# TencentYoutuResearch/ImageMatching-OETR

Hardware: AMD Instinct MI355X
Metric: image-pairs/sec @640x640 (OETR hot path: feature correlation + overlap regression, features resident in HBM) (higher is better)
Workload: dtype f32 (3xf16-split operands, fp32 accumulate); 1 GPU; BASELINE configs[1]: batch=8 pairs/GPU, 640x640 -> 20x20 tokens/image, C=256, 8 enc + 2 dec layers, f32_split_f16; pairs_per_gpu=8, global_pairs=8, streams=3, world_size=1, gpu_max_hw_queues=4, encoder_tile_rows=64, tail_mode=direct form (throughput setting for overlapped streams), parallelism=pairs sharded over 1 rank(s); all-gather of boxes only

## Files before the change

### imagematching_oetr_amd/csrc/api.hip

```cpp
#include <math.h>
#include <stdlib.h>
#include <string.h>

#include <atomic>
#include <string>
#include <vector>

#include "../../include/oetr_hip.h"
#include "../../include/oetr_tail_share.h"
#include "common.h"

using namespace oetr;

constexpr int OETR_PREREDUCE_MIN_TOKENS = 768;
constexpr int OETR_DIRECT_TAIL_MIN_ROWS = 16000;

namespace {

thread_local std::string g_err;

oetr_status fail(oetr_status st, const std::string& msg) {
  g_err = msg;
  return st;
}
// ... 177 lines not shown
}

int encoder_tile_rows(const oetr_ctx* h, const Geom& g) {
  if (!gm_half(h->mode) || h->attn_full) return TM;
  const int want = h->enc_tile;
  if (want == TM || want == 64) return want;
  return g.ntiles > h->num_cus ? 64 : TM;
}
Geom encoder_geom(const Geom& g, int rows) {
  Geom e = g;
  for (int i = 0; i < 2; ++i) e.nt[i] = (g.L[i] + rows - 1) / rows;
  e.tile0[0] = 0; e.tile0[1] = g.N * e.nt[0];
  e.ntiles = g.N * (e.nt[0] + e.nt[1]);
  return e;
}

Workspace carve(const Geom& g, void* base, bool attn_full = false) {
  Workspace w;
  size_t off = 0;
  auto take = [&](size_t floats) {
    float* p = base ? reinterpret_cast<float*>(static_cast<char*>(base) + off) : nullptr;
    off += (floats * sizeof(float) + 255) & ~size_t(255);
    return p;
  };
  const size_t rows = g.rows, nt = g.ntiles;
  w.flags = reinterpret_cast<uint32_t*>(take(OETR_WORKSPACE_STATUS_BYTES / sizeof(float)));
  w.x = take(rows * C);
  w.qp = take((rows + (size_t)2 * g.N * 64) * C);
  w.pos = take((size_t)(g.L[0] + g.L[1]) * C);
  for (int i = 0; i < 2; ++i) { w.kvp[i] = take(nt * KV_FLOATS); w.ksp[i] = take(nt * C); }
  w.att0 = take(nt * C); w.z0 = take(nt * NH);
  w.dkv1 = take(nt * KV_FLOATS); w.dks1 = take(nt * C);
  w.conv_out = take(rows * C);
  w.gn_part = take(nt * 32 * 2);
  w.sm_part = take(nt * 4);
  w.hs = take((size_t)2 * g.N * C);
  w.logits = take(rows);
  w.cxy = take((size_t)2 * g.N * 2);
  w.tlbr = take((size_t)2 * g.N * 4);
  w.convp = take((size_t)9 * rows * C);
  w.kvr = take((size_t)2 * g.N * KV_FLOATS);
  w.ksr = take((size_t)2 * g.N * C);
  for (int i = 0; i < 2; ++i) {
    w.kbuf[i] = attn_full ? take(rows * C) : nullptr;
    w.vt[i] = attn_full ? take((size_t)g.N * C * TM * (g.nt[0] + g.nt[1])) : nullptr;
  }
  w.bytes = off;
  return w;
}

oetr_status check_ws(const Geom& g, void* ws, size_t ws_bytes, Workspace* out, bool attn_full = false) {
  if (!ws) return fail(OETR_ERR_WORKSPACE, "workspace is NULL");
  if (reinterpret_cast<uintptr_t>(ws) & 255)
    return fail(OETR_ERR_WORKSPACE, "workspace must be 256-byte aligned");
  *out = carve(g, ws, attn_full);
  if (out->bytes > ws_bytes)
    return fail(OETR_ERR_WORKSPACE, "workspace too small: need " + std::to_string(out->bytes) +
                                        " bytes, got " + std::to_string(ws_bytes));
  return OETR_OK;
}

HeatLaunch heat_launch(const oetr_ctx* h, const Geom& g, const Workspace& w, const float* mem1,
                       const float* mem2, const float* hs1, const float* hs2, float* cxy1,
                       float* cxy2, int img_h1, int img_h2) {
  HeatLaunch p;
  p.g = g;
  p.w = h->heads;
  p.mem[0] = mem1; p.mem[1] = mem2;
  p.hs[0] = hs1; p.hs[1] = hs2;
  p.conv_out = w.conv_out;
  p.gn_part = w.gn_part;
  p.sm_part = w.sm_part;
  p.logits = w.logits;
  p.cxy[0] = cxy1; p.cxy[1] = cxy2;
  p.img_h[0] = img_h1; p.img_h[1] = img_h2;
  p.tlbr[0] = p.tlbr[1] = nullptr;
  p.box[0] = p.box[1] = nullptr;
  p.img_w[0] = p.img_w[1] = 0;
  p.flags = w.flags;
  p.publish = nullptr;
  p.force_staged_conv = h->tail_mode == 3;
  p.convp_units = 9;
  p.mask[0] = p.mask[1] = nullptr;
  return p;
}

oetr_status check_masks(const oetr_ctx* h, const float* mask1, const float* mask2, bool encoder) {
  if (!mask1 && !mask2) return OETR_OK;
  if (!mask1 || !mask2) return fail(OETR_ERR_BAD_ARG, "masks: pass both mask1 and mask2, or neither");
  if (encoder && ((h->mode != GM_SPLIT && h->mode != GM_F32) || h->attn_full))
    return fail(OETR_ERR_UNSUPPORTED, "masks: built for OETR_DTYPE_F32_SPLIT_F16, OETR_DTYPE_F32_SPLIT_QK16 and OETR_DTYPE_F32 with linear attention "
                                      "(the reference's FullAttention turns a masked query row into NaN, "
                                      "linear_attention.py:74-81)");
  return OETR_OK;
}

struct Scoped {
  oetr_trace* t; hipStream_t s; int slot;
  Scoped(oetr_trace* tr, hipStream_t s_, int kid) : t(tr), s(s_), slot(-1) {
    if (!t) return;
    if (2 * (t->used + 1) > (int)t->ev.size()) { t->dropped++; t = nullptr; return; }
    slot = t->used++;
    t->kid[slot] = kid;
    (void)hipEventRecord(t->ev[2 * slot], s);
  }
  ~Scoped() { if (t) (void)hipEventRecord(t->ev[2 * slot + 1], s); }
};
#define TRACED(h, s, kid, expr)            \
  do {                                     \
    Scoped sc__((h)->trace, s, kid);       \
    HIP_TRY(expr);                         \
  } while (0)

DecLaunch dec_launch(const oetr_ctx* h, const Geom& g, const Workspace& w, bool beside_convp = false) {
  DecLaunch d;
  d.g = encoder_geom(g, encoder_tile_rows(h, g));
  for (int i = 0; i < 2; ++i) { d.layer[i] = h->dec[i]; d.qe[i] = h->qe[i]; }
  d.tgt1 = h->dec_tgt1; d.qkv1 = h->dec_qkv1;
  d.att0_part = w.att0; d.z0_part = w.z0; d.dkv1 = w.dkv1; d.dks1 = w.dks1;
  d.hs = w.hs;
  const int images = 2 * g.N;
  bool fits = images <= DEC_SPLIT_MAX_IMAGES && images * DEC_SPLIT_K * 4 <= h->num_cus;
  d.convp_units = 9;
  if (fits && beside_convp) {
    if (gm_half(h->mode)) {
      const int units = 9 * g.N * ((g.L[0] + RT - 1) / RT + (g.L[1] + RT - 1) / RT);
      const int avail = h->num_cus - images * DEC_SPLIT_K;
      const int upi = std::max(3, (units + avail - 1) / avail);
      fits = upi <= 9;
      if (fits) d.convp_units = upi;
    } else {
      fits = images * DEC_SPLIT_K + g.ntiles <= h->num_cus;
    }
  }
  if (h->dec_split == DEC_SPLIT_K && d.convp_units == 9 && beside_convp && gm_half(h->mode)) d.convp_units = 3;
  d.ksplit = (h->dec_split == DEC_SPLIT_K || (h->dec_split == 0 && fits)) && images <= DEC_SPLIT_MAX_IMAGES
                 ? DEC_SPLIT_K : 1;
  d.flags = w.flags;
  d.xch_epoch = w.flags + STATUS_EPOCH_WORD;
  d.xch = reinterpret_cast<unsigned long long*>(reinterpret_cast<char*>(w.flags) + STATUS_XCH_OFFSET);
  d.tbuf = nullptr;
  d.dbg = 0;
  if (d.ksplit == DEC_SPLIT_K && h->dec_fault) { d.dbg = DEC_DBG_FAULT; h->dec_fault = 0; }
#ifdef OETR_PHASE_TIMING
  d.tbuf = g_tbuf ? g_tbuf + 16 * 4096 : nullptr;
#endif
  return d;
}

oetr_status run_correlation(oetr_ctx* h, const Geom& g, const Workspace& w, const float* feat1,
                            const float* feat2, const float* pos1, const float* pos2,
                            int enc_layers, hipStream_t s, bool with_decoder = true,
                            bool resident = false, const float* mask1 = nullptr,
                            const float* mask2 = nullptr) {
  EncLaunch p;
  memset(&p, 0, sizeof(p));
  if (!resident) {
    p.feat_nchw[0] = feat1; p.feat_nchw[1] = feat2;
    p.pos_nchw[0] = pos1; p.pos_nchw[1] = pos2;
    p.pos_out = w.pos;
  }
  p.tile_rows = encoder_tile_rows(h, g);
  p.g = encoder_geom(g, p.tile_rows);
  p.tail_share = h->tail_share != 0;
  p.attn_full = h->attn_full;
  h->enc_grid.store(encoder_workgroups(p, h->mode), std::memory_order_relaxed);
// ... 1012 lines not shown
oetr_status oetr_debug_mfma_rate(int device, double seconds, double* tflops, void* stream) {
  if (!tflops || !(seconds > 0.0) || seconds > 30.0)
    return fail(OETR_ERR_BAD_ARG, "oetr_debug_mfma_rate: NULL output or seconds outside (0, 30]");
  int ndev = 0;
  if (hipGetDeviceCount(&ndev) != hipSuccess || ndev <= 0 || device < 0 || device >= ndev)
    return fail(OETR_ERR_NO_DEVICE, "no HIP device " + std::to_string(device));
  hipDeviceProp_t prop;
  HIP_TRY(hipGetDeviceProperties(&prop, device));
  int prev = 0;
  (void)hipGetDevice(&prev);
  hipError_t e = hipSetDevice(device);
  if (e == hipSuccess) e = measure_mfma_rate(prop.multiProcessorCount, seconds, tflops, static_cast<hipStream_t>(stream));
  (void)hipSetDevice(prev);
  if (e != hipSuccess) return hip_fail(e, "oetr_debug_mfma_rate");
  return OETR_OK;
}

oetr_status oetr_set_state_prereduce(oetr_handle h, int on) {
  if (!h) return fail(OETR_ERR_BAD_ARG, "oetr_set_state_prereduce: NULL handle");
  if (on < -1 || on > 1) return fail(OETR_ERR_BAD_ARG, "oetr_set_state_prereduce: -1 (auto), 0 (off) or 1 (a reduction launch between the encoder launches)");
  h->kv_prereduce = on;
  return OETR_OK;
}

oetr_status oetr_set_tail_share(oetr_handle h, int mode) {
  if (!h) return fail(OETR_ERR_BAD_ARG, "oetr_set_tail_share: NULL handle");
  if (mode != -1 && mode != 0) return fail(OETR_ERR_BAD_ARG, "oetr_set_tail_share: -1 (auto) or 0 (off)");
  h->tail_share = mode;
  return OETR_OK;
}

int oetr_debug_encoder_grid(oetr_handle h) { return h ? h->enc_grid.load(std::memory_order_relaxed) : -1; }

oetr_status oetr_set_attention(oetr_handle h, oetr_attention mode) {
  if (!h) return fail(OETR_ERR_BAD_ARG, "oetr_set_attention: NULL handle");
  if (mode != OETR_ATTENTION_LINEAR && mode != OETR_ATTENTION_FULL)
    return fail(OETR_ERR_BAD_ARG, "oetr_set_attention: unknown mode");
  if (mode == OETR_ATTENTION_FULL && h->policy != 0)
    return fail(OETR_ERR_UNSUPPORTED, "attention 'full' is not built for OETR_DTYPE_F32_SPLIT_QK16");
  if (mode == OETR_ATTENTION_FULL && !gm_f16_range(h->mode) && h->mode != GM_F32)
    return fail(OETR_ERR_UNSUPPORTED, "attention 'full' is built for OETR_DTYPE_F32_SPLIT_F16, OETR_DTYPE_F16 and OETR_DTYPE_F32");
  h->attn_full = mode == OETR_ATTENTION_FULL;
  return OETR_OK;
}

oetr_status oetr_set_trace(oetr_handle h, oetr_trace_handle t) {
  if (!h) return fail(OETR_ERR_BAD_ARG, "oetr_set_trace: NULL handle");
  h->trace = t;
  return OETR_OK;
}

oetr_status oetr_trace_summary(oetr_trace_handle t, int* n_kernels,
                               const char* names[OETR_TRACE_MAX_KERNELS],
                               int launches[OETR_TRACE_MAX_KERNELS],
                               float total_ms[OETR_TRACE_MAX_KERNELS]) {
  if (!t || !n_kernels || !names || !launches || !total_ms)
    return fail(OETR_ERR_BAD_ARG, "oetr_trace_summary: NULL argument");
  static_assert(K_COUNT <= OETR_TRACE_MAX_KERNELS, "raise OETR_TRACE_MAX_KERNELS");
  for (int i = 0; i < K_COUNT; ++i) { names[i] = kKernelNames[i]; launches[i] = 0; total_ms[i] = 0.f; }
  for (int i = 0; i < t->used; ++i) {
    HIP_TRY(hipEventSynchronize(t->ev[2 * i + 1]));
    float ms = 0.f;
    HIP_TRY(hipEventElapsedTime(&ms, t->ev[2 * i], t->ev[2 * i + 1]));
    launches[t->kid[i]]++;
    total_ms[t->kid[i]] += ms;
  }
  *n_kernels = K_COUNT;
  const int dropped = t->dropped;
  t->used = 0;
  t->dropped = 0;
  if (dropped) return fail(OETR_ERR_BAD_ARG, std::to_string(dropped) + " launches not traced: pool too small");
  return OETR_OK;
}

#ifdef OETR_PHASE_TIMING
int oetr_debug_read_tbuf(long long* host, int n_blocks) {
  if (!g_tbuf) return 1;
  return hipMemcpy(host, g_tbuf, sizeof(long long) * 16 * n_blocks, hipMemcpyDeviceToHost) != hipSuccess;
}
int oetr_debug_read_tbuf_decoder(long long* host, int n_blocks) {
  if (!g_tbuf) return 1;
  return hipMemcpy(host, g_tbuf + 16 * 4096, sizeof(long long) * 16 * n_blocks, hipMemcpyDeviceToHost) != hipSuccess;
}
#endif

}
```

### imagematching_oetr_amd/csrc/common.h

```cpp
#pragma once
#include <hip/hip_runtime.h>
#include <stdint.h>

#include <string>
#include <type_traits>

#include "../../include/oetr_hip.h"

namespace oetr {

constexpr int C = 256;
constexpr int NH = 8;
constexpr int HD = 32;
constexpr int FF = 512;
constexpr int TM = 32;
constexpr int LDA = C + 4;
constexpr int LDH = FF + 4;
constexpr int NTHREADS = 256;
constexpr int KV_FLOATS = NH * HD * HD;
constexpr float LN_EPS = 1e-5f;
constexpr float ATTN_EPS = 1e-6f;
constexpr int MAX_TOKENS = 10000;


// ... 831 lines not shown
  size_t vt_off[2];
  int tile_rows;
  int nwg;
  int tail_share;
  int b_cross;
  int kv_reduced;
  int policy;
  int dbg;
  long long* tbuf;
  uint32_t* flags;
  const float* feat_nchw[2];
  const float* pos_nchw[2];
  float* pos_out;
  const float* mask[2];
};

hipError_t launch_encoder(const EncLaunch& p, bool has_b, int tail, int mode, hipStream_t s);
int encoder_workgroups(const EncLaunch& p, int mode);
hipError_t launch_kv_reduce(const Geom& g, const float* kvp, const float* ksp, float* kvr, float* ksr,
                            hipStream_t s);

struct MhaDev {
  const float *wq_t, *wk_t, *wv_t, *wm_t;
  const float *bq, *bk, *bv;
};
struct DecLayerDev {
  MhaDev self_attn, cross;
  const float *w1_t, *w2_t;
  const float *n1w, *n1b, *n2w, *n2b, *n3w, *n3b;
};
struct DecLaunch {
  Geom g;
  DecLayerDev layer[2];
  const float* qe[2];
  const float* tgt1;
  const float* qkv1;
  const float* att0_part;
  const float* z0_part;
  const float* dkv1;
  const float* dks1;
  float* hs;
  int convp_units;
  int ksplit;
  unsigned long long* xch;
  unsigned* xch_epoch;
  uint32_t* flags;
  long long* tbuf;
  int dbg;
};
struct DecConstLaunch {
  DecLayerDev layer[2];
  const float* qe[2];
  float *tgt1, *q0, *qkv1;
};
hipError_t launch_decoder_consts(const DecConstLaunch& p, hipStream_t s);
hipError_t launch_decoder(const DecLaunch& p, hipStream_t s);

struct HeadsDev {
  const f32x4* conv_w;
  const f32x4* conv_w_l;
  const float *conv_b, *gn_w, *gn_b, *out_w, *out_b;
  const float *tlbr0_t;
  const float *tlbr2_w, *tlbr2_b;
};
struct HeatLaunch {
  Geom g;
  HeadsDev w;
  const float* mem[2];
  const float* hs[2];
  float* conv_out;
  float* gn_part;
  float* sm_part;
  float* logits;
  float* cxy[2];
  int img_h[2];
  float* tlbr[2];
  float* box[2];
  int img_w[2];
  uint32_t* flags;
  uint32_t* publish;
  int force_staged_conv;
  int convp_units;
  const float* mask[2];
};
hipError_t launch_heat_conv(const HeatLaunch& p, int mode, hipStream_t s);
hipError_t launch_heat_conv64(const HeatLaunch& p, int mode, hipStream_t s);
hipError_t launch_decoder_convp(const DecLaunch& d, const HeatLaunch& h, float* P, int mode,
                                hipStream_t s);
hipError_t launch_heat_combine(const HeatLaunch& h, const float* P, hipStream_t s);
hipError_t launch_heat_final(const HeatLaunch& p, hipStream_t s);
hipError_t launch_size_regression(const HeadsDev& w, const float* hs1, const float* hs2,
                                  int n, float* tlbr1, float* tlbr2, hipStream_t s);
hipError_t launch_boxes(const float* cxy, const float* tlbr, int n, int max_h, int max_w,
                        float* box, hipStream_t s);
constexpr int BBC = 1024;
constexpr int NECK_MT = 256;
constexpr int NECK_PIX = 16;
constexpr int NECK_XROW = 2 * C;
constexpr int NECK_RW_MIN_WO = 16;
struct NeckGeom {
  int n_img, hb, wb, ho, wo;
  int HW;
  int rows_in;
  int M;
};
struct NeckProjLaunch {
  NeckGeom g;
  const float* bb;
  const f32x4 *wh[2], *wl[2];
  const float *bias, *ln_w, *ln_b;
  _Float16 *xh, *xl;
  uint32_t* flags;
};
struct NeckConvDesc {
  const f32x4 *wh, *wl;
  const f32x4 *wh_rw, *wl_rw;
  float* part;
  int log2ks, pad, nsplit, nhalf, ncols;
  int item0;
};
struct NeckConvLaunch {
  NeckGeom g;
  const _Float16 *xh, *xl;
  NeckConvDesc conv[3];
  int items_per_mt;
  int mt_rows;
  int row_window;
  int nblocks;
};
struct NeckOutLaunch {
  NeckGeom g;
  const float* part[3];
  int nsplit[3];
  const float* bias[3];
  const f32x4 *wh, *wl;
  const float* bias2;
  float* feat;
  float* tokens;
  uint32_t* flags;
};
hipError_t launch_neck_proj(const NeckProjLaunch& p, hipStream_t s);
hipError_t launch_neck_conv(const NeckConvLaunch& p, hipStream_t s);
int neck_conv_rows(int M, int items_per_mt, int num_cus, int max_rows);
hipError_t launch_neck_out(const NeckOutLaunch& p, hipStream_t s);

hipError_t measure_mfma_rate(int num_cus, double seconds, double* tflops, hipStream_t s);

hipError_t launch_linear_attention(const float* q, const float* k, const float* v, const float* q_mask,
                                   const float* kv_mask, int n, int L, int S, float* out, float* state,
                                   hipStream_t s);
hipError_t launch_full_attention(const float* q, const float* k, const float* v, int n,
                                 int L, int S, float* out, hipStream_t s);
hipError_t launch_full_attention_split(const float* q, const float* k, const float* v, int n,
                                       int L, int S, float* out, uint32_t* flags, hipStream_t s);

}
```

### imagematching_oetr_amd/csrc/heads.hip

```cpp
#include "common.h"

namespace oetr {

constexpr int GN_GROUPS = 32;
constexpr float GN_EPS = 1e-5f;

template <int MODE, int NW>
__global__ __launch_bounds__(64 * NW) void k_heat_conv(HeatLaunch p) {
  constexpr int NT = 8 / NW, THREADS = 64 * NW, WC = 32 * NT;
  constexpr int TPR = THREADS / TM, F4 = 64 / TPR;
  __shared__ __attribute__((aligned(16))) float smem[2 * TILE_FLOATS];
  const Geom& g = p.g;
  const int tid = threadIdx.x, lane = tid & 63, wave = __builtin_amdgcn_readfirstlane(tid >> 6), half = lane >> 5;
  const int col = lane & 31;

  const int logical = xcd_remap(blockIdx.x, g.ntiles);
  const int per = g.nt[0] + g.nt[1];
  const int n = logical / per;
  const int rem = logical - n * per;
  const int side = rem >= g.nt[0];
  const int t_idx = side ? rem - g.nt[0] : rem;
  const int L = g.L[side], hf = g.hf[side], wf = g.wf[side];
  const int l0 = t_idx * TM;
  const int nvalid = min(TM, L - l0);
// ... 242 lines not shown
      }
      d = sum8(d);
      if (hpart == 0 && hr < nhalo) att_s[hr] = d;
    }
  }
  __syncthreads();
  {
    float m = 0.f;
    for (int i = tid; i < nhalo; i += THREADS) m = fmaxf(m, fabsf(att_s[i]));
    m = wave_max(m);
    if (lane == 0) attmax_s[wave] = m;
  }
  __syncthreads();
  float att_scale = 1.0f, att_unscale = 1.0f;
  {
    float m = attmax_s[0];
#pragma unroll
    for (int i = 1; i < THREADS / 64; ++i) m = fmaxf(m, attmax_s[i]);
    if (m > 0.f && m < INFINITY) {
      const int e = ilogbf(m) + 1;
      att_scale = ldexpf(1.0f, -e);
      att_unscale = ldexpf(1.0f, e);
    }
  }
  auto region = [&](int t) { return PlanesT<MODE>(smem + (t & 1) * R_FLOATS, &rg); };
  const int lrow = l0 + hrow;
  const int y = lrow / wf, x = lrow - y * wf;
  auto tap_loads = [&](int tap, f32x4 (&v)[F4], float& att) {
    const int dy = tap / 3 - 1, dx = tap % 3 - 1;
    const int yy = y + dy, xx = x + dx;
    const bool ok = (lrow < L) && (yy >= 0) && (yy < hf) && (xx >= 0) && (xx < wf);
    const int src_row = ok ? yy * wf + xx : 0;
    att = ok ? att_s[src_row - halo0] * att_scale : 0.f;
    const f32x4* mp = reinterpret_cast<const f32x4*>(mem + (size_t)src_row * C) + hpart;
#pragma unroll
    for (int i = 0; i < F4; ++i) v[i] = mp[i * TPR];
  };
  WStream2T<MODE, ROWS> ws;
  ws.set_rows(nvalid);
  ws.set_lane(lane);
  constexpr size_t TAP_UNITS = (size_t)C * C / 8;
  {
    f32x4 v[F4];
    float att;
    tap_loads(0, v, att);
    ws.template prime<C, 0>(p.w.conv_w, p.w.conv_w_l, wave, 0, lane);
    const PlanesT<MODE> first = region(0);
#pragma unroll
    for (int i = 0; i < F4; ++i) first.put4(hrow, 4 * (i * TPR + hpart), v[i] * att);
  }
  __syncthreads();
  f32x16 acc[2] = {f32x16{0}, f32x16{0}};
#pragma unroll 1
  for (int tap = 0; tap < 8; ++tap) {
    f32x4 v[F4];
    float att;
    tap_loads(tap + 1, v, att);
    const PlanesT<MODE> cur = region(tap), nxt = region(tap + 1);
    auto epi = [&](auto CI_) {
      constexpr int CI = decltype(CI_)::value;
      if constexpr (CI % 2 == 1) nxt.put4(hrow, 4 * ((CI / 2) * TPR + hpart), v[CI / 2] * att);
    };
    const f32x4* w = p.w.conv_w + tap * TAP_UNITS;
    const f32x4* wl = p.w.conv_w_l + tap * TAP_UNITS;
    ws.template gemm_epi<C, 0, true, C>(cur, w, wl, wave, 0, lane, acc, w + TAP_UNITS, wl + TAP_UNITS,
                                        wave, 0, epi);
    __syncthreads();
  }
  ws.template gemm<C, 0, false, C>(region(8), p.w.conv_w + 8 * TAP_UNITS, p.w.conv_w_l + 8 * TAP_UNITS, wave, 0, lane,
                                   acc, nullptr, nullptr, 0, 0);
  const float bias = p.w.conv_b[32 * wave + col];
#pragma unroll
  for (int mt = 0; mt < 2; ++mt)
#pragma unroll
    for (int r = 0; r < 16; ++r) acc[mt][r] = fmaf(acc[mt][r], att_unscale, bias);
  range_report<MODE>(rg, p.flags);

  heat_conv64_finish(p, acc, g, side, n, t_idx, nvalid, row_base, lane, wave, half, col);
}

constexpr int HALO_MAX_WF = 40;
constexpr int HALO_MAX_ROWS = RT + 2 * (HALO_MAX_WF + 1);
template <int MODE, int ROWS>
__device__ __forceinline__ void heat_conv64h_body(const HeatLaunch& p, _Float16* planes, float* att_s, float* mask_s,
                                                  float* attmax_s) {
  static_assert(gm_planes(MODE) == 2, "two-plane mode");
  static_assert(16 % WStream2T<MODE, ROWS>::D == 0, "the tap sequence below assumes a ring phase of 0 after every GEMM");
  constexpr int THREADS = 512, TPR = THREADS / RT, F4 = 64 / TPR;
  const Geom& g = p.g;
  const int tid = threadIdx.x, lane = tid & 63, wave = __builtin_amdgcn_readfirstlane(tid >> 6);
  const int half = lane >> 5, col = lane & 31;
  const int nt0 = (g.L[0] + RT - 1) / RT, nt1 = (g.L[1] + RT - 1) / RT;
  const int logical = xcd_remap(blockIdx.x, g.N * (nt0 + nt1));
  const int per = nt0 + nt1;
  const int n = logical / per;
  const int rem = logical - n * per;
  const int side = rem >= nt0;
  const int t_idx = side ? rem - nt0 : rem;
  const int L = g.L[side], wf = g.wf[side];
  const int l0 = t_idx * RT;
  const int nvalid = min(RT, L - l0);
  const float* mem = p.mem[side] + (size_t)n * L * C;
  const size_t row_base = (size_t)g.row0[side] + (size_t)n * L + l0;
  Range rg;
  const int halo0 = l0 - wf - 1, nhalo = RT + 2 * (wf + 1);
  const int hrow = tid / TPR, hpart = tid % TPR;
  constexpr int NPASS = (HALO_MAX_ROWS + RT - 1) / RT;
  f32x4 hv[F4];
  {
    const f32x4* hsp = reinterpret_cast<const f32x4*>(p.hs[side] + (size_t)n * C) + hpart;
#pragma unroll
    for (int i = 0; i < F4; ++i) hv[i] = hsp[i * TPR];
  }
#pragma unroll 1
  for (int ps = 0; ps < NPASS; ++ps) {
    const int hr = ps * RT + hrow;
    const int l = min(max(halo0 + hr, 0), L - 1);
    const f32x4* mp = reinterpret_cast<const f32x4*>(mem + (size_t)l * C) + hpart;
    float d = 0.f;
#pragma unroll
    for (int i = 0; i < F4; ++i) {
      const f32x4 v = mp[i * TPR];
      d += (v[0] * hv[i][0] + v[1] * hv[i][1]) + (v[2] * hv[i][2] + v[3] * hv[i][3]);
    }
    d = sum8(d);
    if (hpart == 0 && hr < nhalo) att_s[hr] = d;
  }
  if (tid < RT) {
    const int l = l0 + tid, x = l - (l / wf) * wf;
    mask_s[tid] = x != 0 ? 1.0f : 0.0f;
    mask_s[RT + tid] = x != wf - 1 ? 1.0f : 0.0f;
  }
  __syncthreads();
  {
    float m = 0.f;
    for (int i = tid; i < nhalo; i += THREADS) m = fmaxf(m, fabsf(att_s[i]));
    m = wave_max(m);
    if (lane == 0) attmax_s[wave] = m;
  }
  __syncthreads();
  float att_scale = 1.0f, att_unscale = 1.0f;
  {
    float m = attmax_s[0];
#pragma unroll
    for (int i = 1; i < THREADS / 64; ++i) m = fmaxf(m, attmax_s[i]);
    if (m > 0.f && m < INFINITY) {
      const int e = ilogbf(m) + 1;
      att_scale = ldexpf(1.0f, -e);
      att_unscale = ldexpf(1.0f, e);
    }
  }
  _Float16* const hi0 = planes;
  _Float16* const lo0 = planes + HALO_MAX_ROWS * LDAH;
  WStream2T<MODE, ROWS> ws;
  ws.set_rows(nvalid);
  ws.set_lane(lane);
  constexpr size_t TAP_UNITS = (size_t)C * C / 8;
  auto tap_of = [](int k) { return 3 * (k % 3) + k / 3; };
  ws.template prime<C, 0>(p.w.conv_w + tap_of(0) * TAP_UNITS, p.w.conv_w_l + tap_of(0) * TAP_UNITS, wave, 0, lane);
  {
    const PlanesT<MODE> H(hi0, lo0, &rg);
#pragma unroll 1
    for (int ps = 0; ps < NPASS; ++ps) {
      const int hr = ps * RT + hrow;
      if (hr < nhalo) {
        const int l = halo0 + hr;
        const bool in = l >= 0 && l < L;
        const float att = in ? att_s[hr] * att_scale : 0.f;
        const f32x4* mp = reinterpret_cast<const f32x4*>(mem + (size_t)min(max(l, 0), L - 1) * C) + hpart;
#pragma unroll
        for (int i = 0; i < F4; ++i) H.put4(hr, 4 * (i * TPR + hpart), mp[i * TPR] * att);
      }
    }
  }
  __syncthreads();
  f32x16 acc[2] = {f32x16{0}, f32x16{0}}, accR[2] = {f32x16{0}, f32x16{0}};
  auto window = [&](int k) {
    const int dy = k % 3 - 1, dx = k / 3 - 1;
    const int shift = (wf + 1) + dy * wf + dx;
    return PlanesT<MODE>(hi0 + shift * LDAH, lo0 + shift * LDAH, &rg);
  };
  auto run = [&](int k, f32x16 (&a)[2], auto HAS_NEXT_) {
    constexpr bool HAS_NEXT = decltype(HAS_NEXT_)::value;
    const int t = tap_of(k), tn = tap_of(HAS_NEXT ? k + 1 : k);
    ws.template gemm<C, 0, HAS_NEXT, C>(window(k), p.w.conv_w + t * TAP_UNITS, p.w.conv_w_l + t * TAP_UNITS, wave, 0, lane,
                                        a, p.w.conv_w + tn * TAP_UNITS, p.w.conv_w_l + tn * TAP_UNITS, wave, 0);
  };
#pragma unroll 1
  for (int k = 0; k < 3; ++k) run(k, acc, std::true_type{});
#pragma unroll
  for (int mt = 0; mt < 2; ++mt)
#pragma unroll
    for (int r = 0; r < 16; ++r) acc[mt][r] *= mask_s[32 * mt + crow(r, half)];
#pragma unroll 1
  for (int k = 3; k < 6; ++k) run(k, acc, std::true_type{});
#pragma unroll 1
  for (int k = 6; k < 8; ++k) run(k, accR, std::true_type{});
  run(8, accR, std::false_type{});
  const float bias = p.w.conv_b[32 * wave + col];
#pragma unroll
  for (int mt = 0; mt < 2; ++mt)
#pragma unroll
    for (int r = 0; r < 16; ++r)
      acc[mt][r] = fmaf(fmaf(accR[mt][r], mask_s[RT + 32 * mt + crow(r, half)], acc[mt][r]), att_unscale, bias);
  range_report<MODE>(rg, p.flags);
  heat_conv64_finish(p, acc, g, side, n, t_idx, nvalid, row_base, lane, wave, half, col);
}

template <int MODE>
__global__ __launch_bounds__(512) void k_heat_conv64(HeatLaunch p) {
  __shared__ __attribute__((aligned(16))) float smem[2 * R_FLOATS];
  __shared__ float att_s[RT + 2 * (100 + 1) + 6];
  __shared__ float attmax_s[512 / 64];
  const Geom& g = p.g;
  const int nt0 = (g.L[0] + RT - 1) / RT, nt1 = (g.L[1] + RT - 1) / RT;
  if ((int)blockIdx.x >= g.N * (nt0 + nt1)) return size_reg_body(p, blockIdx.x - g.N * (nt0 + nt1), smem);
  const int logical = xcd_remap(blockIdx.x, g.N * (nt0 + nt1));
  const int rem = logical - (logical / (nt0 + nt1)) * (nt0 + nt1);
  const int side = rem >= nt0;
  const int t_idx = side ? rem - nt0 : rem;
  const int nvalid = min(RT, g.L[side] - t_idx * RT);
  if (__builtin_amdgcn_readfirstlane(nvalid > 32 ? 1 : 0)) heat_conv64_body<MODE, 2>(p, smem, att_s, attmax_s);
  else heat_conv64_body<MODE, 1>(p, smem, att_s, attmax_s);
}

template <int MODE>
__global__ __launch_bounds__(512) void k_heat_conv64h(HeatLaunch p) {
  __shared__ __attribute__((aligned(16))) _Float16 planes[2 * HALO_MAX_ROWS * LDAH];
  __shared__ float att_s[HALO_MAX_ROWS + 6];
  __shared__ float mask_s[2 * RT];
  __shared__ float attmax_s[512 / 64];
  const Geom& g = p.g;
  const int nt0 = (g.L[0] + RT - 1) / RT, nt1 = (g.L[1] + RT - 1) / RT;
  if ((int)blockIdx.x >= g.N * (nt0 + nt1))
    return size_reg_body(p, blockIdx.x - g.N * (nt0 + nt1), reinterpret_cast<float*>(planes));
  const int logical = xcd_remap(blockIdx.x, g.N * (nt0 + nt1));
  const int rem = logical - (logical / (nt0 + nt1)) * (nt0 + nt1);
  const int side = rem >= nt0;
  const int t_idx = side ? rem - nt0 : rem;
  const int nvalid = min(RT, g.L[side] - t_idx * RT);
  if (__builtin_amdgcn_readfirstlane(nvalid > 32 ? 1 : 0)) heat_conv64h_body<MODE, 2>(p, planes, att_s, mask_s, attmax_s);
  else heat_conv64h_body<MODE, 1>(p, planes, att_s, mask_s, attmax_s);
}

hipError_t launch_heat_conv64(const HeatLaunch& p, int mode, hipStream_t s) {
  if (mode != GM_SPLIT) return hipErrorInvalidValue;
  const int tiles = p.g.N * ((p.g.L[0] + RT - 1) / RT + (p.g.L[1] + RT - 1) / RT);
  if (p.g.wf[0] <= HALO_MAX_WF && p.g.wf[1] <= HALO_MAX_WF && !p.force_staged_conv)
    hipLaunchKernelGGL((k_heat_conv64h<GM_SPLIT>), dim3(tiles + 2 * p.g.N), dim3(512), 0, s, p);
  else
    hipLaunchKernelGGL((k_heat_conv64<GM_SPLIT>), dim3(tiles + 2 * p.g.N), dim3(512), 0, s, p);
  return hipGetLastError();
}

__global__ __launch_bounds__(512) void k_heat_combine(HeatLaunch p, const float* __restrict__ P) {
  constexpr int TPR = 16, F4 = 4;
  __shared__ __attribute__((aligned(16))) float out_s[TM * LDA];
  __shared__ float att_s[TM + 2 * (100 + 1) + 6];
  const Geom& g = p.g;
  const int tid = threadIdx.x;
  if ((int)blockIdx.x >= g.ntiles) return size_reg_body(p, blockIdx.x - g.ntiles, out_s);
  const int logical = xcd_remap(blockIdx.x, g.ntiles);
  const int per = g.nt[0] + g.nt[1];
  const int n = logical / per;
  const int rem = logical - n * per;
  const int side = rem >= g.nt[0];
  const int t_idx = side ? rem - g.nt[0] : rem;
  const int L = g.L[side], hf = g.hf[side], wf = g.wf[side];
  const int l0 = t_idx * TM;
  const int nvalid = min(TM, L - l0);
  const int slot = g.tile0[side] + n * g.nt[side] + t_idx;
  const float* mem = p.mem[side] + (size_t)n * L * C;
  const size_t img_row0 = (size_t)g.row0[side] + (size_t)n * L;
  const int halo0 = l0 - wf - 1, nhalo = TM + 2 * (wf + 1);
  const int hrow = tid / TPR, hpart = tid % TPR;
  {
    const f32x4* hsp = reinterpret_cast<const f32x4*>(p.hs[side] + (size_t)n * C) + hpart;
    f32x4 hv[F4];
#pragma unroll
    for (int i = 0; i < F4; ++i) hv[i] = hsp[i * TPR];
    for (int r0 = 0; r0 < nhalo; r0 += TM) {
      const int hr = r0 + hrow;
      const int l = min(max(halo0 + hr, 0), L - 1);
      const f32x4* mp = reinterpret_cast<const f32x4*>(mem + (size_t)l * C) + hpart;
      float d = 0.f;
#pragma unroll
      for (int i = 0; i < F4; ++i) {
        const f32x4 v = mp[i * TPR];
        d += (v[0] * hv[i][0] + v[1] * hv[i][1]) + (v[2] * hv[i][2] + v[3] * hv[i][3]);
      }
      d = sum8(d);
      d += dpp_mov<0x140>(d);
      if (hpart == 0 && hr < nhalo) att_s[hr] = d;
    }
  }
  __syncthreads();
  {
    const int l = l0 + hrow;
    const int y = l / wf, x = l - y * wf;
    f32x4 acc[F4];
#pragma unroll
    for (int i = 0; i < F4; ++i) acc[i] = reinterpret_cast<const f32x4*>(p.w.conv_b)[i * TPR + hpart];
#pragma unroll
    for (int tap = 0; tap < 9; ++tap) {
      const int dy = tap / 3 - 1, dx = tap % 3 - 1;
      const int yy = y + dy, xx = x + dx;
      const bool ok = (l < L) && (yy >= 0) && (yy < hf) && (xx >= 0) && (xx < wf);
      const int src_row = ok ? yy * wf + xx : 0;
      const float att = ok ? att_s[src_row - halo0] : 0.f;
      const f32x4* pp = reinterpret_cast<const f32x4*>(
                            P + ((size_t)tap * g.rows + img_row0 + src_row) * C) + hpart;
#pragma unroll
      for (int i = 0; i < F4; ++i) acc[i] += pp[i * TPR] * att;
    }
    f32x4* go = reinterpret_cast<f32x4*>(p.conv_out + (img_row0 + min(l, L - 1)) * C) + hpart;
#pragma unroll
    for (int i = 0; i < F4; ++i) {
      if (l < L) go[i * TPR] = acc[i];
      *reinterpret_cast<f32x4*>(out_s + hrow * LDA + 4 * (i * TPR + hpart)) = acc[i];
    }
  }
  __syncthreads();
  if (tid < 256) {
    const int grp = tid >> 3, rs = tid & 7;
    float s = 0.f;
// ... 240 lines not shown
```

Measured before the change: 34680 image-pairs/s.

## Apply attention weights per tap after GEMM instead of pre-scaling halo planes

The halo conv kernel no longer multiplies the staged feature rows by the attention value before splitting them into f16 planes. It builds a per-tap, per-output-row scale table (attention of the source row times the border validity) and applies it to a separate per-tap GEMM accumulator. This removes the max-reduction pass, its two barriers and the power-of-two scale. It also merges the halo loads so memory is read once for both the dot product and staging, and adds phase-timing stamps under a debug macro. In exchange it adds a 9-tap scale FMA epilogue and extra accumulator registers, and puts raw features instead of rescaled ones into the f16 split planes.

```diff
diff --git a/imagematching_oetr_amd/csrc/api.hip b/imagematching_oetr_amd/csrc/api.hip
--- a/imagematching_oetr_amd/csrc/api.hip
+++ b/imagematching_oetr_amd/csrc/api.hip
@@ -283,6 +283,9 @@
   p.force_staged_conv = h->tail_mode == 3;
   p.convp_units = 9;
   p.mask[0] = p.mask[1] = nullptr;
+#ifdef OETR_PHASE_TIMING
+  p.tbuf = g_tbuf ? g_tbuf + 16 * 8192 : nullptr;
+#endif
   return p;
 }
 
@@ -1461,6 +1464,10 @@
   if (!g_tbuf) return 1;
   return hipMemcpy(host, g_tbuf + 16 * 4096, sizeof(long long) * 16 * n_blocks, hipMemcpyDeviceToHost) != hipSuccess;
 }
+int oetr_debug_read_tbuf_heads(long long* host, int n_blocks) {
+  if (!g_tbuf) return 1;
+  return hipMemcpy(host, g_tbuf + 16 * 8192, sizeof(long long) * 16 * n_blocks, hipMemcpyDeviceToHost) != hipSuccess;
+}
 #endif
 
 }
diff --git a/imagematching_oetr_amd/csrc/common.h b/imagematching_oetr_amd/csrc/common.h
--- a/imagematching_oetr_amd/csrc/common.h
+++ b/imagematching_oetr_amd/csrc/common.h
@@ -937,6 +937,9 @@
   int force_staged_conv;
   int convp_units;
   const float* mask[2];
+#ifdef OETR_PHASE_TIMING
+  long long* tbuf;
+#endif
 };
 hipError_t launch_heat_conv(const HeatLaunch& p, int mode, hipStream_t s);
 hipError_t launch_heat_conv64(const HeatLaunch& p, int mode, hipStream_t s);
diff --git a/imagematching_oetr_amd/csrc/heads.hip b/imagematching_oetr_amd/csrc/heads.hip
--- a/imagematching_oetr_amd/csrc/heads.hip
+++ b/imagematching_oetr_amd/csrc/heads.hip
@@ -348,10 +348,10 @@
 constexpr int HALO_MAX_WF = 40;
 constexpr int HALO_MAX_ROWS = RT + 2 * (HALO_MAX_WF + 1);
 template <int MODE, int ROWS>
-__device__ __forceinline__ void heat_conv64h_body(const HeatLaunch& p, _Float16* planes, float* att_s, float* mask_s,
-                                                  float* attmax_s) {
+__device__ __forceinline__ void heat_conv64h_body(const HeatLaunch& p, _Float16* planes, float* att_s, float* scale_s) {
   static_assert(gm_planes(MODE) == 2, "two-plane mode");
   static_assert(16 % WStream2T<MODE, ROWS>::D == 0, "the tap sequence below assumes a ring phase of 0 after every GEMM");
+  static_assert(RT == 64, "the scale table below is written one tap per wave, one output row per lane");
   constexpr int THREADS = 512, TPR = THREADS / RT, F4 = 64 / TPR;
   const Geom& g = p.g;
   const int tid = threadIdx.x, lane = tid & 63, wave = __builtin_amdgcn_readfirstlane(tid >> 6);
@@ -363,114 +363,102 @@
   const int rem = logical - n * per;
   const int side = rem >= nt0;
   const int t_idx = side ? rem - nt0 : rem;
-  const int L = g.L[side], wf = g.wf[side];
+  const int L = g.L[side], hf = g.hf[side], wf = g.wf[side];
   const int l0 = t_idx * RT;
   const int nvalid = min(RT, L - l0);
   const float* mem = p.mem[side] + (size_t)n * L * C;
   const size_t row_base = (size_t)g.row0[side] + (size_t)n * L + l0;
   Range rg;
+  PHASE_STAMP(p, 0);
   const int halo0 = l0 - wf - 1, nhalo = RT + 2 * (wf + 1);
   const int hrow = tid / TPR, hpart = tid % TPR;
-  constexpr int NPASS = (HALO_MAX_ROWS + RT - 1) / RT;
-  f32x4 hv[F4];
-  {
-    const f32x4* hsp = reinterpret_cast<const f32x4*>(p.hs[side] + (size_t)n * C) + hpart;
-#pragma unroll
-    for (int i = 0; i < F4; ++i) hv[i] = hsp[i * TPR];
-  }
-#pragma unroll 1
-  for (int ps = 0; ps < NPASS; ++ps) {
-    const int hr = ps * RT + hrow;
-    const int l = min(max(halo0 + hr, 0), L - 1);
-    const f32x4* mp = reinterpret_cast<const f32x4*>(mem + (size_t)l * C) + hpart;
-    float d = 0.f;
-#pragma unroll
-    for (int i = 0; i < F4; ++i) {
-      const f32x4 v = mp[i * TPR];
-      d += (v[0] * hv[i][0] + v[1] * hv[i][1]) + (v[2] * hv[i][2] + v[3] * hv[i][3]);
-    }
-    d = sum8(d);
-    if (hpart == 0 && hr < nhalo) att_s[hr] = d;
-  }
-  if (tid < RT) {
-    const int l = l0 + tid, x = l - (l / wf) * wf;
-    mask_s[tid] = x != 0 ? 1.0f : 0.0f;
-    mask_s[RT + tid] = x != wf - 1 ? 1.0f : 0.0f;
-  }
-  __syncthreads();
-  {
-    float m = 0.f;
-    for (int i = tid; i < nhalo; i += THREADS) m = fmaxf(m, fabsf(att_s[i]));
-    m = wave_max(m);
-    if (lane == 0) attmax_s[wave] = m;
-  }
-  __syncthreads();
-  float att_scale = 1.0f, att_unscale = 1.0f;
-  {
-    float m = attmax_s[0];
-#pragma unroll
-    for (int i = 1; i < THREADS / 64; ++i) m = fmaxf(m, attmax_s[i]);
-    if (m > 0.f && m < INFINITY) {
-      const int e = ilogbf(m) + 1;
-      att_scale = ldexpf(1.0f, -e);
-      att_unscale = ldexpf(1.0f, e);
-    }
-  }
   _Float16* const hi0 = planes;
   _Float16* const lo0 = planes + HALO_MAX_ROWS * LDAH;
   WStream2T<MODE, ROWS> ws;
   ws.set_rows(nvalid);
   ws.set_lane(lane);
   constexpr size_t TAP_UNITS = (size_t)C * C / 8;
-  auto tap_of = [](int k) { return 3 * (k % 3) + k / 3; };
-  ws.template prime<C, 0>(p.w.conv_w + tap_of(0) * TAP_UNITS, p.w.conv_w_l + tap_of(0) * TAP_UNITS, wave, 0, lane);
+  constexpr int NPASS = (HALO_MAX_ROWS + RT - 1) / RT;
+  f32x4 hv[F4], v[NPASS][F4];
+  {
+    const f32x4* hsp = reinterpret_cast<const f32x4*>(p.hs[side] + (size_t)n * C) + hpart;
+#pragma unroll
+    for (int i = 0; i < F4; ++i) hv[i] = hsp[i * TPR];
+  }
+#pragma unroll
+  for (int ps = 0; ps < NPASS; ++ps) {
+    if (ps * RT >= nhalo) break;
+    const int l = min(max(halo0 + ps * RT + hrow, 0), L - 1);
+    const f32x4* mp = reinterpret_cast<const f32x4*>(mem + (size_t)l * C) + hpart;
+#pragma unroll
+    for (int i = 0; i < F4; ++i) v[ps][i] = mp[i * TPR];
+  }
+  ws.template prime<C, 0>(p.w.conv_w, p.w.conv_w_l, wave, 0, lane);
   {
     const PlanesT<MODE> H(hi0, lo0, &rg);
-#pragma unroll 1
+#pragma unroll
     for (int ps = 0; ps < NPASS; ++ps) {
+      if (ps * RT >= nhalo) break;
       const int hr = ps * RT + hrow;
+      float d = 0.f;
+#pragma unroll
+      for (int i = 0; i < F4; ++i)
+        d += (v[ps][i][0] * hv[i][0] + v[ps][i][1] * hv[i][1]) + (v[ps][i][2] * hv[i][2] + v[ps][i][3] * hv[i][3]);
+      d = sum8(d);
       if (hr < nhalo) {
-        const int l = halo0 + hr;
-        const bool in = l >= 0 && l < L;
-        const float att = in ? att_s[hr] * att_scale : 0.f;
-        const f32x4* mp = reinterpret_cast<const f32x4*>(mem + (size_t)min(max(l, 0), L - 1) * C) + hpart;
-#pragma unroll
-        for (int i = 0; i < F4; ++i) H.put4(hr, 4 * (i * TPR + hpart), mp[i * TPR] * att);
+        if (hpart == 0) att_s[hr] = d;
+#pragma unroll
+        for (int i = 0; i < F4; ++i) H.put4(hr, 4 * (i * TPR + hpart), v[ps][i]);
       }
     }
   }
-  __syncthreads();
-  f32x16 acc[2] = {f32x16{0}, f32x16{0}}, accR[2] = {f32x16{0}, f32x16{0}};
-  auto window = [&](int k) {
-    const int dy = k % 3 - 1, dx = k / 3 - 1;
-    const int shift = (wf + 1) + dy * wf + dx;
-    return PlanesT<MODE>(hi0 + shift * LDAH, lo0 + shift * LDAH, &rg);
-  };
-  auto run = [&](int k, f32x16 (&a)[2], auto HAS_NEXT_) {
+  PHASE_STAMP(p, 1);
+  __syncthreads();
+  {
+    const int l = l0 + lane, y = l / wf, x = l - y * wf;
+    for (int tap = wave; tap < 9; tap += THREADS / 64) {
+      const int dy = tap / 3 - 1, dx = tap - 3 * (tap / 3) - 1;
+      const bool ok = l < L && y + dy >= 0 && y + dy < hf && x + dx >= 0 && x + dx < wf;
+      scale_s[tap * RT + lane] = ok ? att_s[(wf + 1) + lane + dy * wf + dx] : 0.f;
+    }
+  }
+  __syncthreads();
+  PHASE_STAMP(p, 2);
+  f32x16 acc[2] = {f32x16{0}, f32x16{0}};
+  auto run = [&](int k, auto HAS_NEXT_) {
     constexpr bool HAS_NEXT = decltype(HAS_NEXT_)::value;
-    const int t = tap_of(k), tn = tap_of(HAS_NEXT ? k + 1 : k);
-    ws.template gemm<C, 0, HAS_NEXT, C>(window(k), p.w.conv_w + t * TAP_UNITS, p.w.conv_w_l + t * TAP_UNITS, wave, 0, lane,
-                                        a, p.w.conv_w + tn * TAP_UNITS, p.w.conv_w_l + tn * TAP_UNITS, wave, 0);
+    const int shift = (wf + 1) + (k / 3 - 1) * wf + (k - 3 * (k / 3) - 1);
+    const int kn = HAS_NEXT ? k + 1 : k;
+    f32x16 acc_tap[2] = {f32x16{0}, f32x16{0}};
+    ws.template gemm<C, 0, HAS_NEXT, C>(PlanesT<MODE>(hi0 + shift * LDAH, lo0 + shift * LDAH, &rg), p.w.conv_w + k * TAP_UNITS,
+                                        p.w.conv_w_l + k * TAP_UNITS, wave, 0, lane, acc_tap, p.w.conv_w + kn * TAP_UNITS,
+                                        p.w.conv_w_l + kn * TAP_UNITS, wave, 0);
+    const float* sc = scale_s + k * RT + 4 * half;
+#pragma unroll
+    for (int mt = 0; mt < ROWS; ++mt)
+#pragma unroll
+      for (int j = 0; j < 4; ++j) {
+        const f32x4 s = *reinterpret_cast<const f32x4*>(sc + 32 * mt + 8 * j);
+#pragma unroll
+        for (int q = 0; q < 4; ++q) acc[mt][4 * j + q] = fmaf(s[q], acc_tap[mt][4 * j + q], acc[mt][4 * j + q]);
+      }
   };
 #pragma unroll 1
-  for (int k = 0; k < 3; ++k) run(k, acc, std::true_type{});
+  for (int k = 0; k < 8; ++k) {
+    run(k, std::true_type{});
+    if (k == 2) PHASE_STAMP(p, 3);
+    if (k == 5) PHASE_STAMP(p, 4);
+  }
+  run(8, std::false_type{});
+  PHASE_STAMP(p, 5);
+  const float bias = p.w.conv_b[32 * wave + col];
 #pragma unroll
   for (int mt = 0; mt < 2; ++mt)
 #pragma unroll
-    for (int r = 0; r < 16; ++r) acc[mt][r] *= mask_s[32 * mt + crow(r, half)];
-#pragma unroll 1
-  for (int k = 3; k < 6; ++k) run(k, acc, std::true_type{});
-#pragma unroll 1
-  for (int k = 6; k < 8; ++k) run(k, accR, std::true_type{});
-  run(8, accR, std::false_type{});
-  const float bias = p.w.conv_b[32 * wave + col];
-#pragma unroll
-  for (int mt = 0; mt < 2; ++mt)
-#pragma unroll
-    for (int r = 0; r < 16; ++r)
-      acc[mt][r] = fmaf(fmaf(accR[mt][r], mask_s[RT + 32 * mt + crow(r, half)], acc[mt][r]), att_unscale, bias);
+    for (int r = 0; r < 16; ++r) acc[mt][r] += bias;
   range_report<MODE>(rg, p.flags);
   heat_conv64_finish(p, acc, g, side, n, t_idx, nvalid, row_base, lane, wave, half, col);
+  PHASE_STAMP(p, 6);
 }
 
 template <int MODE>
@@ -494,8 +482,7 @@
 __global__ __launch_bounds__(512) void k_heat_conv64h(HeatLaunch p) {
   __shared__ __attribute__((aligned(16))) _Float16 planes[2 * HALO_MAX_ROWS * LDAH];
   __shared__ float att_s[HALO_MAX_ROWS + 6];
-  __shared__ float mask_s[2 * RT];
-  __shared__ float attmax_s[512 / 64];
+  __shared__ __attribute__((aligned(16))) float scale_s[9 * RT];
   const Geom& g = p.g;
   const int nt0 = (g.L[0] + RT - 1) / RT, nt1 = (g.L[1] + RT - 1) / RT;
   if ((int)blockIdx.x >= g.N * (nt0 + nt1))
@@ -505,8 +492,8 @@
   const int side = rem >= nt0;
   const int t_idx = side ? rem - nt0 : rem;
   const int nvalid = min(RT, g.L[side] - t_idx * RT);
-  if (__builtin_amdgcn_readfirstlane(nvalid > 32 ? 1 : 0)) heat_conv64h_body<MODE, 2>(p, planes, att_s, mask_s, attmax_s);
-  else heat_conv64h_body<MODE, 1>(p, planes, att_s, mask_s, attmax_s);
+  if (__builtin_amdgcn_readfirstlane(nvalid > 32 ? 1 : 0)) heat_conv64h_body<MODE, 2>(p, planes, att_s, scale_s);
+  else heat_conv64h_body<MODE, 1>(p, planes, att_s, scale_s);
 }
 
 hipError_t launch_heat_conv64(const HeatLaunch& p, int mode, hipStream_t s) {
```

Result: no change. 34710 image-pairs/s, median of 4 (+0.1%).
